# zprodev/zlib.es

Hardware: AMD Instinct MI355X
Metric: GiB/s deflate+inflate round trip, 64 MiB buffers (uncompressed bytes / wall), bit-exact vs reference (higher is better)
Workload: dtype u8; 1 GPU; random64: 1 x 64 MiB xorshift buffer(s) per GPU (seed 12345+index), deflate then inflate, HBM-resident; bytes_per_buffer=67108864, compressed_bytes=67176156, parallelism=independent buffers, one per GPU

## Files before the change

### zlib.es_amd/csrc/zes_api.hip

```cpp
#include "../../include/zes.h"
#include "zes_kernels.h"
#include "zes_chain.h"

#include <algorithm>
#include <atomic>
#include <condition_variable>
#include <cstdio>
#include <cstddef>
#include <cstdlib>
#include <cstring>
#include <chrono>
#include <functional>
#include <future>
#include <initializer_list>
#include <deque>
#include <map>
#include <mutex>
#include <string>
#include <thread>
#include <vector>

extern "C" int zes_gen(uint8_t* out, uint64_t n, uint32_t kind, uint32_t seed);

namespace {
// ... 694 lines not shown
                       ZES_SORT_MODE_FIRST | (use_index ? ZES_SORT_USE_INDEX : 0u));
  }
  auto note = [&](uint32_t* flag_to, uint32_t* word_to) -> int {
    HIPCHK(hipMemcpyAsync(flag_to, idx_a + ZES_BLK - 1, 4, hipMemcpyDeviceToHost, g.stream));
    if (word_to) HIPCHK(hipMemcpyAsync(word_to, idx_b + ZES_BLK - 1, 4, hipMemcpyDeviceToHost, g.stream));
    return ZES_OK;
  };
  if (route && (rc = note(&route[0], &route[3]))) return rc;
  if (use_index) {
    {
      Timed t("k_lz_index");
      hipLaunchKernelGGL(k_lz_index, dim3(grid), dim3(IDX_THREADS), 0, g.stream, d_in, dbufs, dblks, idx_a, idx_b, idx_a, (uint16_t*)g.sdelta.p);
    }
    if (route && (rc = note(&route[1], &route[4]))) return rc;
    {
      Timed t("k_lz_sort_redo");
      hipLaunchKernelGGL(k_lz_sort, dim3(grid), dim3(SORT_THREADS), 0, g.stream, d_in, dbufs, dblks, idx_a, idx_b, idx_a, (uint16_t*)g.sdelta.p,
                         ZES_SORT_MODE_REDO);
    }
    if (route && (rc = note(&route[2], nullptr))) return rc;
  }
  if ((rc = after_index())) return rc;
  {
    Timed t("k_lz_match");
    hipLaunchKernelGGL(k_lz_match, dim3(grid), dim3(MATCH_THREADS), 0, g.stream, d_in, dbufs, dblks, idx_a, idx_b, (uint32_t*)g.mlist.p);
  }
  if (phases && (rc = phases_arm(zes_lazy_set_dbg, grid))) return rc;
  {
    const uint32_t* order = nullptr;
    if (heaviest_first) {
      if ((rc = ensure(g.order, (size_t)grid * 4))) return rc;
      Timed t("k_lz_order");
      hipLaunchKernelGGL(k_lz_order, dim3(1), dim3(1024), 0, g.stream, (const uint32_t*)idx_a, grid, (uint32_t*)g.order.p);
      order = (const uint32_t*)g.order.p;
    }
    Timed t("k_lz_match_lazy");
    hipLaunchKernelGGL(k_lz_match_lazy, dim3(grid), dim3(MATCH_THREADS), 0, g.stream, d_in, dbufs, dblks, idx_a, (const uint32_t*)idx_a,
                       (const uint16_t*)g.sdelta.p, idx_b, (uint32_t*)g.tmask.p, (uint32_t*)g.mlist.p, order);
  }
  if (phases) {
    if ((rc = phases_print(zes_lazy_set_dbg, grid, 5,
                           "zes lazy match steps (avg cycles over %u blocks): stage %.0f tail %.0f window chains %.0f entry chains %.0f true chain (only unmerged blocks) %.0f | first wave, window chains: %.0f loop turns\n")))
      return rc;
    if ((rc = phases_arm(zes_parse_set_dbg, grid))) return rc;
  }
  {
    Timed t("k_lz_parse_small");
    hipLaunchKernelGGL(k_lz_parse_small, dim3(grid), dim3(PARSE_THREADS), 0, g.stream, d_in, dbufs, dblks, idx_b, idx_a, (uint32_t*)g.hists.p,
                       (const uint32_t*)g.tmask.p, (const uint32_t*)g.mlist.p);
  }
  {
    Timed t("k_lz_parse");
    hipLaunchKernelGGL(k_lz_parse, dim3(grid), dim3(PARSE_THREADS), 0, g.stream, d_in, dbufs, dblks, idx_b, idx_a, (uint32_t*)g.hists.p,
                       (const uint32_t*)g.tmask.p, (const uint32_t*)g.mlist.p);
  }
  return ZES_OK;
}

struct DeflateRange {
  uint64_t n_read = 0;
  uint32_t flags = 0;
  uint32_t start_bit = 0;
  bool defer = false;
  uint32_t adler = 1;
};

int deflate_batch_core(const uint8_t* d_in, const uint64_t* in_off, const uint64_t* in_len, uint8_t* d_out,
                       const uint64_t* out_off, const uint64_t* out_cap, uint64_t* out_len, int32_t* status,
                       uint32_t count, DeflateRange* one = nullptr) {
  std::vector<ZesBuf> hb;
  uint64_t nblk_total = 0;
  std::vector<uint32_t> live;
  hb.reserve(count);
  for (uint32_t i = 0; i < count; i++) {
    out_len[i] = 0;
    if (deflate_throws(in_len[i])) {
      status[i] = ZES_E_CORRUPT;
      continue;
    }
    if (out_cap[i] < deflate_bound(in_len[i])) {
      status[i] = ZES_E_NOSPACE;
      out_len[i] = deflate_bound(in_len[i]);
      continue;
    }
    if ((out_off[i] & 15u) || (((uintptr_t)d_out) & 15u)) {
      status[i] = ZES_E_ARG;
      continue;
    }
    status[i] = ZES_OK;
    ZesBuf b;
    b.in_off = in_off[i];
    b.n = in_len[i];
    b.out_off = out_off[i];
    b.cap = out_cap[i];
    b.first_blk = (uint32_t)nblk_total;
    b.nblk = (uint32_t)((in_len[i] + ZES_BLK - 1) / ZES_BLK);
    b.n_read = one ? std::max(one->n_read, in_len[i]) : in_len[i];
    b.flags = one ? one->flags : 0u;
    b.start_bit = one ? one->start_bit : 0u;
    nblk_total += b.nblk;
    hb.push_back(b);
    live.push_back(i);
  }
  if (hb.empty()) return ZES_OK;
  if (nblk_total >= (1ull << 31)) return ZES_E_ARG;
  const uint32_t nbuf = (uint32_t)hb.size(), nblk = (uint32_t)nblk_total;
  int rc;
  if ((rc = ensure(g.bufs, sizeof(ZesBuf) * nbuf))) return rc;
  if ((rc = ensure(g.blks, sizeof(ZesBlk) * nblk))) return rc;
  if ((rc = ensure(g.idx_a, (size_t)nblk * ZES_BLK * 4))) return rc;
  if ((rc = ensure(g.idx_b, (size_t)nblk * ZES_BLK * 4))) return rc;
  if ((rc = ensure(g.sdelta, (size_t)nblk * ZES_BLK * 2 + 64))) return rc;
  if ((rc = ensure(g.tmask, (size_t)nblk * ZES_TMASK_WORDS * 4))) return rc;
  if ((rc = ensure(g.mlist, (size_t)nblk * ZES_MLIST_WORDS * 4))) return rc;
  if ((rc = ensure(g.hists, (size_t)nblk * 320 * 4))) return rc;
  if ((rc = ensure(g.codes, (size_t)nblk * 320 * 4))) return rc;
  if ((rc = ensure(g.hdrs, (size_t)nblk * ZES_HDR_WORDS * 4))) return rc;
  if ((rc = ensure(g.adler, (size_t)nbuf * 16))) return rc;
  if ((rc = ensure(g.res, sizeof(ZesRes) * nbuf))) return rc;
  ZesBuf* dbufs = (ZesBuf*)g.bufs.p;
  ZesBlk* dblks = (ZesBlk*)g.blks.p;
  unsigned long long* adler = (unsigned long long*)g.adler.p;
  if (nbuf > 1) {
    if (nbuf <= DEFLATE_TABLE_BUFS) {
      memcpy(g.pinned->def.table, hb.data(), sizeof(ZesBuf) * nbuf);
      HIPCHK(hipMemcpyAsync(g.bufs.p, g.pinned->def.table, sizeof(ZesBuf) * nbuf, hipMemcpyHostToDevice, g.stream));
    } else {
      HIPCHK(hipMemcpy(g.bufs.p, hb.data(), sizeof(ZesBuf) * nbuf, hipMemcpyHostToDevice));
    }
  }
  {
    Timed t("k_make_blks");
    const uint32_t nthr = std::max(nblk, 2u * nbuf);
    hipLaunchKernelGGL(k_make_blks, dim3((nthr + 255) / 256), dim3(256), 0, g.stream, hb[0], nbuf, dbufs, dblks, nblk, adler);
  }
  {
    HIPCHK(hipEventRecord(g.ev_a0, g.stream));
    HIPCHK(hipStreamWaitEvent(g.s_adler, g.ev_a0, 0));
    Timed t("k_adler", g.s_adler);
    if (nbuf == 1) {
      const uint32_t nch = (uint32_t)((hb[0].n + ADLER_CHUNK - 1) / ADLER_CHUNK);
      hipLaunchKernelGGL(k_adler, dim3(nch), dim3(ADLER_THREADS), 0, g.s_adler, d_in, hb[0].in_off, hb[0].n, adler);
    } else {
      hipLaunchKernelGGL(k_adler_blocks, dim3(nblk), dim3(ADLER_THREADS), 0, g.s_adler, d_in, dbufs, dblks, adler);
    }
  }
  HIPCHK(hipEventRecord(g.ev_a1, g.s_adler));
  const bool sort_dbg = getenv("ZES_DEBUG_PHASES") != nullptr;
  if (sort_dbg && (rc = phases_arm(zes_sort_set_dbg, nblk))) return rc;
  static const bool use_index = getenv("ZES_NO_INDEX") == nullptr;
  rc = launch_lz77(d_in, nblk, use_index, nbuf > 1 && nblk > 256, sort_dbg, [&]() -> int {
    if (!sort_dbg) return ZES_OK;
    return phases_print(zes_sort_set_dbg, nblk, 7,
                        "zes sort steps (avg cycles over %u blocks): zero %.0f count %.0f flag %.0f compact %.0f stage %.0f three passes %.0f sd/inv %.0f\n");
  });
  if (rc) return rc;
  if (sort_dbg) {
    if ((rc = phases_print(zes_parse_set_dbg, nblk, 7, "zes parse steps (avg cycles over %u blocks): A %.0f B %.0f C %.0f D1 %.0f D2 %.0f D3 %.0f out %.0f\n"))) return rc;
    if ((rc = phases_arm(zes_huff_set_dbg, nblk))) return rc;
  }
  ZesRes* res_direct = (nbuf <= DEFLATE_DIRECT_BUFS && g.pinned_dev) ? g.pinned_dev->def.res : nullptr;
  {
    Timed t("k_huff");
    hipLaunchKernelGGL(k_huff, dim3(nblk), dim3(HUFF_THREADS_HOST), 0, g.stream, dblks, (const uint32_t*)g.hists.p,
                       (uint32_t*)g.codes.p, (uint32_t*)g.hdrs.p);
  }
  if (sort_dbg && (rc = phases_print(zes_huff_set_dbg, nblk, 7,
                                     "zes huff steps (avg cycles over %u blocks): rank sorts %.0f both alphabets' levels %.0f codes %.0f run-length coding %.0f its code %.0f header bits %.0f totals+out %.0f\n")))
    return rc;
  {
    HIPCHK(hipStreamWaitEvent(g.stream, g.ev_a1, 0));
    Timed t("k_layout");
    hipLaunchKernelGGL(k_layout, dim3(nbuf), dim3(256), 0, g.stream, d_out, dbufs, dblks, adler, res_direct ? res_direct : (ZesRes*)g.res.p);
  }
  {
    Timed t("k_emit");
    hipLaunchKernelGGL(k_emit, dim3(nblk), dim3(EMIT_THREADS), 0, g.stream, d_out, dbufs, dblks, (uint32_t*)g.idx_a.p,
                       (const uint32_t*)g.codes.p, (const uint32_t*)g.hdrs.p);
  }
  HIPCHK(hipGetLastError());
  ZesRes* r = g.pinned->def.res;
  if (nbuf > DEFLATE_DIRECT_BUFS) {
    if (nbuf > g.res_more_n) {
      if (g.res_more) HIPCHK(hipHostFree(g.res_more));
      g.res_more = nullptr;
      g.res_more_n = 0;
      HIPCHK(hipHostMalloc((void**)&g.res_more, sizeof(ZesRes) * nbuf * 2, hipHostMallocDefault));
      g.res_more_n = (size_t)nbuf * 2;
    }
    r = g.res_more;
  }
  if (!res_direct) HIPCHK(hipMemcpyAsync(r, g.res.p, sizeof(ZesRes) * nbuf, hipMemcpyDeviceToHost, g.stream));
  if (one && one->defer) return ZES_OK;
  HIPCHK(hipStreamSynchronize(g.stream));
  collect_times();
  for (uint32_t k = 0; k < nbuf; k++) {
    out_len[live[k]] = r[k].out_len;
    status[live[k]] = r[k].status;
  }
  if (one) one->adler = r[0].aux;
  return ZES_OK;
}

int deflate_one(const uint8_t* d_in, uint64_t in_off, uint64_t n, uint8_t* d_out, uint64_t out_off, uint64_t cap, uint64_t* out_len,
                DeflateRange* range = nullptr) {
  int32_t st = 0;
  const int rc = deflate_batch_core(d_in, &in_off, &n, d_out, &out_off, &cap, out_len, &st, 1, range);
  return rc ? rc : st;
}

int read_res(ZesRes* out) {
  HIPCHK(hipMemcpyAsync(&g.pinned->res1, g.res.p, sizeof(ZesRes), hipMemcpyDeviceToHost, g.stream));
  HIPCHK(hipStreamSynchronize(g.stream));
  *out = g.pinned->res1;
  return ZES_OK;
}

struct InfJob {
  uint64_t in_off, c, out_off, cap;
  uint64_t out_len;
  int status;
  int tier;
  uint32_t start0 = 16, hist = 0;
  bool partial = false, final_seen = false;
  uint64_t end_bit = 0;
  int btype0 = -1;
  bool want_end = false;
};

ZesInfBuf inf_buf(const InfJob& j) {
  ZesInfBuf b;
  memset(&b, 0, sizeof b);
  b.in_off = j.in_off;
  b.c = j.c;
  b.out_off = j.out_off;
  b.cap = j.cap;
  return b;
}

bool t1_eligible(const InfJob& j, uint32_t flags) { return !(flags & (ZES_F_NO_FASTPATH | ZES_F_PIECES)) && j.c >= 64 && j.c < (1ull << 29); }

int launch_verify(const uint8_t* d_in, const ZesInfBuf* dbufs, uint32_t surv_cap, uint32_t* counters, uint32_t* cnt, uint32_t loose,
                  uint64_t total_c) {
  int rc;
  const uint32_t vlong_cap = (uint32_t)std::min<uint64_t>(total_c / 256 + 4096, surv_cap);
  if ((rc = ensure(g.vlong, (size_t)vlong_cap * 24))) return rc;
  uint32_t nwg = (uint32_t)std::min<uint64_t>(total_c / 16384 + 1, 8192);
  if (const char* e = getenv("ZES_VERIFY_DIV")) nwg = (uint32_t)std::min<uint64_t>(total_c / (uint64_t)atoi(e) + 1, 8192);
  {
    Timed t("k_inf_verify");
    hipLaunchKernelGGL(k_inf_verify, dim3(nwg), dim3(64), 0, g.stream, d_in, dbufs, (const unsigned long long*)g.surv.p, surv_cap, counters,
                       (uint32_t*)g.cand.p, cnt, loose, (uint32_t*)g.vlong.p, vlong_cap,
                       getenv("ZES_VERIFY_STEPS") ? (uint32_t)atoi(getenv("ZES_VERIFY_STEPS")) : 32u);
  }
  {
    Timed t("k_inf_verify_long");
    const uint32_t nlong = (uint32_t)std::min<uint64_t>(total_c / 2048 + 1, 32768);
    hipLaunchKernelGGL(k_inf_verify_long, dim3(nlong), dim3(64), 0, g.stream, d_in, dbufs, (const unsigned long long*)g.surv.p, surv_cap,
                       counters, (uint32_t*)g.cand.p, cnt, loose, (const uint32_t*)g.vlong.p, vlong_cap);
  }
  if (getenv("ZES_VERIFY_DBG")) {
    uint32_t hc[4];
    HIPCHK(hipStreamSynchronize(g.stream));
    HIPCHK(hipMemcpy(hc, counters, 16, hipMemcpyDeviceToHost));
    fprintf(stderr, "verify: survivors %u, handed to the wave form %u\n", hc[0], hc[1]);
  }
  return ZES_OK;
}

void host_lap(const char* what) {
  static const bool on = getenv("ZES_DEBUG_HOSTLAPS") != nullptr;
  if (!on) return;
  static thread_local std::chrono::steady_clock::time_point last = std::chrono::steady_clock::now();
  const auto now = std::chrono::steady_clock::now();
  fprintf(stderr, "zes host lap: %-34s %8.1f us\n", what, std::chrono::duration<double, std::micro>(now - last).count());
  last = now;
}

int print_par_phases(const unsigned long long* dbg, uint64_t work) {
    std::vector<unsigned long long> h((size_t)work * ZES_PAR_DBG_ROW);
    HIPCHK(hipMemcpy(h.data(), dbg, h.size() * 8, hipMemcpyDeviceToHost));
    double acc[8] = {0}, t0[3] = {0}, t15[3] = {0}, fb_lanes = 0, fb_waves = 0, hs[5] = {0}, p4[5] = {0}, why[3] = {0};
    uint32_t cntd = 0;
    for (uint32_t i = 0; i < work; i++) {
      const unsigned long long* r = &h[(size_t)i * ZES_PAR_DBG_ROW];
      if (!r[7]) continue;
      cntd++;
      for (int k = 1; k < 8; k++) acc[k] += (double)(r[k] - r[k - 1]);
      for (int k = 0; k < 3; k++) {
        t0[k] += (double)(r[8 + k] - r[1]);
        t15[k] += (double)(r[12 + k] - r[1]);
      }
      hs[0] += (double)(r[16] - r[0]);
      for (int k = 1; k < 5; k++) hs[k] += (double)(r[16 + k] - r[15 + k]);
      for (int k = 0; k < 5; k++) p4[k] += (double)r[24 + k];
      fb_lanes += (double)r[11];
      fb_waves += (double)r[15];
      for (int k = 0; k < 3; k++) why[k] += (double)r[29 + k];
    }
    fprintf(stderr, "zes phases (avg cycles over %u blocks): hdr %.0f tables %.0f compose %.0f count %.0f emit %.0f resolve %.0f flush %.0f\n",
            cntd, acc[1] / cntd, acc[2] / cntd, acc[3] / cntd, acc[4] / cntd, acc[5] / cntd, acc[6] / cntd, acc[7] / cntd);
    fprintf(stderr, "zes table steps, cycles since the header: first wave window %.0f landing %.0f fill %.0f | last wave %.0f %.0f %.0f\n",
            t0[0] / cntd, t0[1] / cntd, t0[2] / cntd, t15[0] / cntd, t15[1] / cntd, t15[2] / cntd);
    fprintf(stderr, "zes header steps (avg cycles): staging %.0f fixed fields + code-length code %.0f code lengths %.0f lit/len tables %.0f distance tables %.0f\n",
            hs[0] / cntd, hs[1] / cntd, hs[2] / cntd, hs[3] / cntd, hs[4] / cntd);
    fprintf(stderr, "zes resolve steps (avg cycles): carry+clear %.0f fill %.0f jumping %.0f copy %.0f | %.1f barrier rounds per block\n", p4[0] / cntd,
            p4[1] / cntd, p4[2] / cntd, p4[3] / cntd, p4[4] / cntd);
// ... 4723 lines not shown
```

### zlib.es_amd/csrc/zes_deflate.hip

```cpp
#include "zes_common.h"
#include "zes_kernels.h"

__device__ static inline uint32_t lds_ld32u(const uint8_t* s, uint32_t off) {
  const uint32_t* w = reinterpret_cast<const uint32_t*>(s);
  uint32_t i = off >> 2;
  uint32_t lo = w[i], hi = w[i + 1];
  return __builtin_amdgcn_alignbyte(hi, lo, off & 3u);
}

__device__ static inline void stage_block(uint8_t* s, const uint8_t* g, uint32_t bytes, uint32_t padded) {
  const uint32_t tid = threadIdx.x, nth = blockDim.x;
  const uint32_t mis = (uint32_t)((uintptr_t)g & 15u);
  if (mis == 0) {
    const uint4* g4 = reinterpret_cast<const uint4*>(g);
    uint4* s4 = reinterpret_cast<uint4*>(s);
    const uint32_t full = bytes >> 4;
    for (uint32_t i = tid; i < full; i += nth) s4[i] = g4[i];
    for (uint32_t i = (full << 4) + tid; i < padded; i += nth) s[i] = i < bytes ? g[i] : (uint8_t)0;
  } else {
    for (uint32_t i = tid; i < padded; i += nth) s[i] = i < bytes ? g[i] : (uint8_t)0;
  }
}

__device__ unsigned long long* g_sort_dbg = nullptr;
void zes_sort_set_dbg(unsigned long long* p) { (void)hipMemcpyToSymbol(HIP_SYMBOL(g_sort_dbg), &p, sizeof p); }
#define SSTAMP(i)                                                                                        \
  do {                                                                                                   \
    if (g_sort_dbg && threadIdx.x == 0) g_sort_dbg[(size_t)blockIdx.x * 8 + (i)] = (unsigned long long)clock64(); \
  } while (0)

#define SORT_HASH_BITS 19u
#define SORT_OWN 128u
#ifndef SORT_ROUNDS
#define SORT_ROUNDS 8u
#endif
#define SORT_TILE (SORT_THREADS * SORT_ROUNDS)
static_assert(SORT_ROUNDS == 4u || SORT_ROUNDS == 8u || SORT_ROUNDS == 16u, "the arrival wait names four, eight or sixteen registers");
struct SortSmem {
  uint8_t in[ZES_BLK + 16];
  uint32_t hist[3][256];
  uint32_t base[2][256];
  uint16_t whist[2][SORT_WAVES][256];
  uint32_t wsum[SORT_WAVES];
  uint32_t nsat;
  uint32_t heavy;
};
static_assert((1u << SORT_HASH_BITS) * 2u / 8u <= ZES_BLK, "counter table must fit the block area");
static_assert(SORT_OWN * SORT_THREADS == ZES_BLK, "one thread per 128 positions");

__device__ __forceinline__ static uint32_t sort_hash(uint32_t key24) { return (key24 * 0x9E3779B1u) >> (32u - SORT_HASH_BITS); }
__device__ __forceinline__ static uint32_t sort_hash2(uint32_t key24) { return ((key24 ^ (key24 >> 11)) * 0xC2B2AE35u) >> (32u - SORT_HASH_BITS); }

__device__ __forceinline__ static uint4 sort_ld16(const uint8_t* __restrict__ src, bool aligned, uint32_t off, uint32_t T) {
  if (aligned && off + 16u <= T) return *reinterpret_cast<const uint4*>(src + off);
  uint32_t t[4] = {0, 0, 0, 0};
  for (uint32_t k = 0; k < 16u; k++)
    if (off + k < T) t[k >> 2] |= (uint32_t)src[off + k] << (8u * (k & 3u));
  return make_uint4(t[0], t[1], t[2], t[3]);
}

__global__ __launch_bounds__(SORT_THREADS) void k_lz_sort(const uint8_t* __restrict__ d_in, const ZesBuf* __restrict__ bufs,
                                                          const ZesBlk* __restrict__ blks, uint32_t* idx_a,
                                                          uint32_t* __restrict__ idx_b, uint32_t* inv_all, uint16_t* __restrict__ sd_all,
                                                          uint32_t mode) {
  __shared__ __align__(16) SortSmem S;
  const uint32_t g = blockIdx.x, tid = threadIdx.x, lane = tid & 63u, wave = tid >> 6;
  const ZesBlk bk = blks[g];
  const ZesBuf bf = bufs[bk.buf];
  const uint32_t T = bk.len;
  const uint8_t* src = d_in + bf.in_off + (uint64_t)bk.blk * ZES_BLK;
  uint32_t* A = idx_a + (uint64_t)g * ZES_BLK;
  uint32_t* B = idx_b + (uint64_t)g * ZES_BLK;
  const uint32_t cnt = T >= 3 ? T - 2 : 0;
  const bool redo = (mode & 0xffu) == ZES_SORT_MODE_REDO;
  if (redo && !(A[ZES_BLK - 1] & ZES_SORT_REDO)) return;
  if (cnt == 0) {
    if (tid == 0) A[ZES_BLK - 1] = 0;
    return;
  }

  SSTAMP(0);
  uint32_t* tbl = reinterpret_cast<uint32_t*>(S.in);
  {
    uint4* t4 = reinterpret_cast<uint4*>(S.in);
    for (uint32_t i = tid; i < ZES_BLK / 16; i += SORT_THREADS) t4[i] = make_uint4(0, 0, 0, 0);
    for (uint32_t i = tid; i < 4 * 3 * 256; i += SORT_THREADS) reinterpret_cast<uint32_t*>(&S.whist[0][0][0])[i] = 0;
    if (tid == 0) {
      S.nsat = 0;
      S.heavy = 0;
    }
  }
  __syncthreads();
  SSTAMP(1);
  const bool aligned = (((uintptr_t)src) & 15u) == 0;
  const uint32_t p0 = tid * SORT_OWN;
  uint32_t samp[SORT_OWN / 16];
#pragma unroll
  for (uint32_t c = 0; c < SORT_OWN / 16; c++) samp[c] = ~0u;
  if (p0 < cnt && !redo) {
    uint4 cur = sort_ld16(src, aligned, p0, T);
#pragma unroll 1
    for (uint32_t c = 0; c < SORT_OWN / 16; c++) {
      const uint4 nxt = sort_ld16(src, aligned, p0 + 16u * (c + 1u), T);
      const uint32_t w[5] = {cur.x, cur.y, cur.z, cur.w, nxt.x};
#pragma unroll
      for (uint32_t k = 0; k < 16; k++) {
        const uint32_t key = __builtin_amdgcn_alignbyte(w[(k >> 2) + 1], w[k >> 2], k & 3u) & 0xffffffu;
        const uint32_t h = sort_hash(key);
        const uint32_t sh = (h & 15u) * 2u;
        const bool inr = p0 + 16u * c + k < cnt;
        const bool sat = (tbl[h >> 4] >> sh) & 2u;
        if (k == 0 && inr) {
#pragma unroll
          for (uint32_t cc = 0; cc < SORT_OWN / 16; cc++) samp[cc] = (cc == c) ? h : samp[cc];
        }
        if (inr && !sat) {
          const uint32_t old = atomicOr(&tbl[h >> 4], 1u << sh);
          if (((old >> sh) & 3u) == 1u) atomicOr(&tbl[h >> 4], 2u << sh);
        }
      }
      cur = nxt;
    }
  }
  __syncthreads();
  SSTAMP(2);
  {
    uint32_t kept = 0, tried = 0;
#pragma unroll
    for (uint32_t c = 0; c < SORT_OWN / 16; c++) {
      const uint32_t h = samp[c];
      if (h != ~0u) {
        tried++;
        kept += (tbl[h >> 4] >> ((h & 15u) * 2u + 1u)) & 1u;
      }
    }
    atomicAdd(&S.nsat, kept | (tried << 16));
  }
  __syncthreads();
  const bool dense = redo || (S.nsat & 0xFFFFu) * 4u >= (S.nsat >> 16) * 3u;
#ifndef NO_LAZY
  if (dense && !redo && (mode & ZES_SORT_USE_INDEX) && inv_all != nullptr) {
    uint32_t* cc = reinterpret_cast<uint32_t*>(&S.whist[0][0][0]);
    {
      uint32_t ky[SORT_OWN / 16];
#pragma unroll
      for (uint32_t c = 0; c < SORT_OWN / 16; c++) {
        const uint32_t sp = min(p0 + 16u * c + (((tid * 8u + c) * 0x9E3779B1u) >> 28), T >= 8u ? T - 8u : 0u);
        uint32_t w = 0, w2 = 0;
        if (T >= 8u) {
          __builtin_memcpy(&w, src + (sp & ~3u), 4);
          __builtin_memcpy(&w2, src + (sp & ~3u) + 4u, 4);
        }
        ky[c] = __builtin_amdgcn_alignbyte(w2, w, sp & 3u) & 0xffffffu;
      }
#pragma unroll
      for (uint32_t c = 0; c < SORT_OWN / 16; c++)
        if (p0 + 16u * c < cnt) atomicAdd(&cc[sort_hash(ky[c]) >> (SORT_HASH_BITS - 11u)], 1u);
    }
    __syncthreads();
    {
      const uint32_t thr = max(2u, (32u * cnt + (ZES_BLK - 1u)) >> 17);
      const uint32_t a = cc[2u * tid], b = cc[2u * tid + 1u];
      const uint32_t w = (a > thr ? a : 0u) + (b > thr ? b : 0u);
      if (w) atomicAdd(&S.heavy, w);
    }
    __syncthreads();
    if (S.heavy * 256u <= cnt) {
      if (tid == 0) A[ZES_BLK - 1] = cnt | ZES_SORT_LAZY | ZES_SORT_INDEX;
      return;
    }
    cc[2u * tid] = 0;
    cc[2u * tid + 1u] = 0;
    __syncthreads();
  }
#endif
  const bool two = !redo && (S.nsat & 0xFFFFu) * 5u < (S.nsat >> 16) * 2u;
  if (tid == 0) B[ZES_BLK - 1] = (two ? ZES_ROUTE_SORT_TWO : 0u) | (dense ? ZES_ROUTE_SORT_DENSE : 0u);
  uint32_t ns = cnt;
  if (!dense) {
  uint32_t f0 = 0, f1 = 0, f2 = 0, f3 = 0;
  uint32_t(*sub)[256] = reinterpret_cast<uint32_t(*)[256]>(&S.whist[0][0][0]) + 3u * (lane & 3u);
  if (p0 < cnt) {
    uint4 cur = sort_ld16(src, aligned, p0, T);
#pragma unroll 1
    for (uint32_t c = 0; c < SORT_OWN / 16; c++) {
      const uint4 nxt = sort_ld16(src, aligned, p0 + 16u * (c + 1u), T);
      const uint32_t w[5] = {cur.x, cur.y, cur.z, cur.w, nxt.x};
      uint32_t bits = 0;
#pragma unroll
      for (uint32_t k = 0; k < 16; k++) {
        const uint32_t key = __builtin_amdgcn_alignbyte(w[(k >> 2) + 1], w[k >> 2], k & 3u) & 0xffffffu;
        const uint32_t h = sort_hash(key);
        const uint32_t keep = (tbl[h >> 4] >> ((h & 15u) * 2u + 1u)) & 1u;
        if (keep && p0 + 16u * c + k < cnt) {
          bits |= 1u << k;
          if (!two) {
            atomicAdd(&sub[0][(key >> 16) & 255u], 1u);
            atomicAdd(&sub[1][(key >> 8) & 255u], 1u);
            atomicAdd(&sub[2][key & 255u], 1u);
          }
        }
      }
      const uint32_t v = bits << (16u * (c & 1u));
      f0 |= (c >> 1) == 0u ? v : 0u;
      f1 |= (c >> 1) == 1u ? v : 0u;
      f2 |= (c >> 1) == 2u ? v : 0u;
      f3 |= (c >> 1) == 3u ? v : 0u;
      cur = nxt;
    }
  }
  if (two) {
    __syncthreads();
    {
      uint4* t4 = reinterpret_cast<uint4*>(S.in);
      for (uint32_t i = tid; i < ZES_BLK / 16; i += SORT_THREADS) t4[i] = make_uint4(0, 0, 0, 0);
    }
    __syncthreads();
    if (p0 < cnt) {
      uint4 cur = sort_ld16(src, aligned, p0, T);
#pragma unroll 1
      for (uint32_t c = 0; c < SORT_OWN / 16; c++) {
        const uint4 nxt = sort_ld16(src, aligned, p0 + 16u * (c + 1u), T);
        const uint32_t w[5] = {cur.x, cur.y, cur.z, cur.w, nxt.x};
        const uint32_t fw = (c >> 1) == 0u ? f0 : (c >> 1) == 1u ? f1 : (c >> 1) == 2u ? f2 : f3;
        const uint32_t bits = (fw >> (16u * (c & 1u))) & 0xffffu;
#pragma unroll
        for (uint32_t k = 0; k < 16; k++) {
          const uint32_t key = __builtin_amdgcn_alignbyte(w[(k >> 2) + 1], w[k >> 2], k & 3u) & 0xffffffu;
          const uint32_t h = sort_hash2(key);
          const uint32_t sh = (h & 15u) * 2u;
          if ((bits >> k) & 1u) {
            const uint32_t old = atomicOr(&tbl[h >> 4], 1u << sh);
            if (((old >> sh) & 3u) == 1u) atomicOr(&tbl[h >> 4], 2u << sh);
          }
        }
        cur = nxt;
      }
    }
    __syncthreads();
    if (p0 < cnt) {
      uint32_t g0 = 0, g1 = 0, g2 = 0, g3 = 0;
      uint4 cur = sort_ld16(src, aligned, p0, T);
#pragma unroll 1
      for (uint32_t c = 0; c < SORT_OWN / 16; c++) {
        const uint4 nxt = sort_ld16(src, aligned, p0 + 16u * (c + 1u), T);
        const uint32_t w[5] = {cur.x, cur.y, cur.z, cur.w, nxt.x};
        const uint32_t fw = (c >> 1) == 0u ? f0 : (c >> 1) == 1u ? f1 : (c >> 1) == 2u ? f2 : f3;
        const uint32_t bits = (fw >> (16u * (c & 1u))) & 0xffffu;
        uint32_t nb = 0;
#pragma unroll
        for (uint32_t k = 0; k < 16; k++) {
          const uint32_t key = __builtin_amdgcn_alignbyte(w[(k >> 2) + 1], w[k >> 2], k & 3u) & 0xffffffu;
          const uint32_t h = sort_hash2(key);
          const uint32_t keep = (tbl[h >> 4] >> ((h & 15u) * 2u + 1u)) & 1u;
          if (keep && ((bits >> k) & 1u)) {
            nb |= 1u << k;
            atomicAdd(&sub[0][(key >> 16) & 255u], 1u);
            atomicAdd(&sub[1][(key >> 8) & 255u], 1u);
            atomicAdd(&sub[2][key & 255u], 1u);
          }
        }
        const uint32_t v = nb << (16u * (c & 1u));
        g0 |= (c >> 1) == 0u ? v : 0u;
        g1 |= (c >> 1) == 1u ? v : 0u;
        g2 |= (c >> 1) == 2u ? v : 0u;
        g3 |= (c >> 1) == 3u ? v : 0u;
        cur = nxt;
      }
      f0 = g0;
      f1 = g1;
      f2 = g2;
      f3 = g3;
    }
  }
  SSTAMP(3);
  const uint32_t mine = (uint32_t)(__popc(f0) + __popc(f1) + __popc(f2) + __popc(f3));
  uint32_t incl = mine;
#pragma unroll
  for (int d = 1; d < 64; d <<= 1) {
    const uint32_t t = __shfl_up(incl, d);
    if ((int)lane >= d) incl += t;
  }
  if (lane == 63) S.wsum[wave] = incl;
  __syncthreads();
  uint32_t woff = 0;
  ns = 0;
#pragma unroll
  for (uint32_t w = 0; w < SORT_WAVES; w++) {
    const uint32_t v = S.wsum[w];
    woff += w < wave ? v : 0u;
    ns += v;
  }
  uint32_t* fbits = reinterpret_cast<uint32_t*>(S.in);
  uint32_t* fpre = reinterpret_cast<uint32_t*>(S.in) + 4096;
  if (two) {
    uint32_t o = woff + incl - mine;
#pragma unroll
    for (uint32_t w = 0; w < 4; w++) {
      uint32_t f = w == 0u ? f0 : w == 1u ? f1 : w == 2u ? f2 : f3;
      while (f) {
        B[o++] = p0 + 32u * w + (uint32_t)__builtin_ctz(f);
        f &= f - 1u;
      }
    }
  } else {
    uint32_t o = woff + incl - mine;
    fbits[4 * tid + 0] = f0;
    fpre[4 * tid + 0] = o;
    o += (uint32_t)__popc(f0);
    fbits[4 * tid + 1] = f1;
    fpre[4 * tid + 1] = o;
    o += (uint32_t)__popc(f1);
    fbits[4 * tid + 2] = f2;
    fpre[4 * tid + 2] = o;
    o += (uint32_t)__popc(f2);
    fbits[4 * tid + 3] = f3;
    fpre[4 * tid + 3] = o;
  }
  if (tid < 3 * 256) {
    const uint32_t* hs = reinterpret_cast<const uint32_t*>(&S.whist[0][0][0]);
    (&S.hist[0][0])[tid] = hs[tid] + hs[768 + tid] + hs[1536 + tid] + hs[2304 + tid];
  }
  __syncthreads();
  if (!two) {
    for (uint32_t p = tid; p < cnt; p += SORT_THREADS) {
      const uint32_t w = fbits[p >> 5];
      if ((w >> (p & 31u)) & 1u) B[fpre[p >> 5] + (uint32_t)__popc(w & ((1u << (p & 31u)) - 1u))] = p;
    }
  }
  }
  __syncthreads();
  SSTAMP(4);
#ifdef NO_LAZY
  const bool lazy = false;
#else
  const bool lazy = inv_all != nullptr && ns * 2u >= cnt;
#endif
  if (tid == 0) A[ZES_BLK - 1] = ns | (lazy ? ZES_SORT_LAZY : 0u);
  if (ns == 0) return;

  stage_block(S.in, src, T, (T + 15u) & ~15u);
  __syncthreads();
  if (dense) {
    uint32_t(*hc)[256] = reinterpret_cast<uint32_t(*)[256]>(&S.whist[0][0][0]);
    for (uint32_t i = tid; i < T; i += SORT_THREADS) atomicAdd(&hc[lane & 3u][S.in[i]], 1u);
    __syncthreads();
    if (tid < 256) {
      const uint32_t H = hc[0][tid] + hc[1][tid] + hc[2][tid] + hc[3][tid];
#pragma unroll
      for (uint32_t ps = 0; ps < 3; ps++) {
        const uint32_t off = 2u - ps;
        uint32_t h = H;
        for (uint32_t e = 0; e < off; e++) h -= (S.in[e] == tid);
        for (uint32_t e = off + cnt; e < T; e++) h -= (S.in[e] == tid);
        S.hist[ps][tid] = h;
      }
    }
    __syncthreads();
  }
  SSTAMP(5);

  uint32_t bsel = 0;
  for (int pass = 0; pass < 3; pass++) {
    const uint32_t off = 2u - (uint32_t)pass;
    const uint32_t* from = (pass == 1) ? A : B;
    uint32_t* to = (pass == 1) ? B : A;
    {
      uint32_t* w0 = reinterpret_cast<uint32_t*>(&S.whist[0][wave][0]);
      w0[lane] = 0;
      w0[lane + 64u] = 0;
    }
    if (wave == 0) {
      uint32_t c[4];
      uint32_t sum = 0;
#pragma unroll
      for (int k = 0; k < 4; k++) {
        c[k] = S.hist[pass][lane * 4 + k];
        sum += c[k];
      }
      uint32_t in2 = sum;
#pragma unroll
      for (int d = 1; d < 64; d <<= 1) {
        const uint32_t t = __shfl_up(in2, d);
        if ((int)lane >= d) in2 += t;
      }
      uint32_t run = in2 - sum;
#pragma unroll
      for (int k = 0; k < 4; k++) {
        S.base[bsel][lane * 4 + k] = run;
        run += c[k];
      }
    }
    __syncthreads();
    const uint32_t ntiles = (ns + SORT_TILE - 1) / SORT_TILE;
    uint32_t pn[SORT_ROUNDS];
#pragma unroll
    for (uint32_t r = 0; r < SORT_ROUNDS; r++) pn[r] = from[min(wave * (SORT_TILE / SORT_WAVES) + lane + 64u * r, ns - 1u)];
    for (uint32_t t = 0; t < ntiles; t++) {
      uint16_t(*wh)[256] = S.whist[t & 1];
      const uint32_t i0 = t * SORT_TILE + wave * (SORT_TILE / SORT_WAVES) + lane;
      uint32_t p[SORT_ROUNDS], d[SORT_ROUNDS], rk[SORT_ROUNDS];
#pragma unroll
      for (uint32_t r = 0; r < SORT_ROUNDS; r++) p[r] = (dense && pass == 0) ? min(i0 + 64u * r, ns - 1u) : pn[r];
      asm volatile("" : "+v"(p[0]), "+v"(p[1]), "+v"(p[2]), "+v"(p[3]));
#if SORT_ROUNDS >= 8u
      asm volatile("" : "+v"(p[4]), "+v"(p[5]), "+v"(p[6]), "+v"(p[7]));
#endif
#if SORT_ROUNDS == 16u
      asm volatile("" : "+v"(p[8]), "+v"(p[9]), "+v"(p[10]), "+v"(p[11]));
      asm volatile("" : "+v"(p[12]), "+v"(p[13]), "+v"(p[14]), "+v"(p[15]));
#endif
#pragma unroll
      for (uint32_t r = 0; r < SORT_ROUNDS; r++) d[r] = (i0 + 64u * r < ns) ? S.in[p[r] + off] : 0u;
      uint32_t* wrow = reinterpret_cast<uint32_t*>(&wh[wave][0]);
#pragma unroll
      for (uint32_t r = 0; r < SORT_ROUNDS; r++) {
        const bool valid = i0 + 64u * r < ns;
        const uint32_t sh = 16u * (d[r] & 1u);
        const uint32_t old = valid ? atomicAdd(&wrow[d[r] >> 1], 1u << sh) : 0u;
        rk[r] = (old >> sh) & 0xffffu;
      }
      __syncthreads();
      if (tid < 256) {
        uint32_t c[SORT_WAVES];
#pragma unroll
        for (int w = 0; w < SORT_WAVES; w++) c[w] = wh[w][tid];
        uint32_t o = 0;
#pragma unroll
        for (int w = 0; w < SORT_WAVES; w++) {
          wh[w][tid] = (uint16_t)o;
          o += c[w];
        }
        S.base[bsel ^ 1][tid] = S.base[bsel][tid] + o;
      }
      __syncthreads();
      {
        uint32_t* wnext = reinterpret_cast<uint32_t*>(&S.whist[(t + 1u) & 1u][wave][0]);
        wnext[lane] = 0;
        wnext[lane + 64u] = 0;
      }
#pragma unroll
      for (uint32_t r = 0; r < SORT_ROUNDS; r++) pn[r] = from[min(i0 + SORT_TILE + 64u * r, ns - 1u)];
#pragma unroll
      for (uint32_t r = 0; r < SORT_ROUNDS; r++) {
        const uint32_t dst = S.base[bsel][d[r]] + wh[wave][d[r]] + rk[r];
        const bool valid = i0 + 64u * r < ns;
        to[valid ? dst : ZES_BLK - 2u] = p[r];
      }
      bsel ^= 1;
    }
    __syncthreads();
    SSTAMP(6);
  }
  if (lazy) {
    uint32_t* inv = inv_all + (uint64_t)g * ZES_BLK;
    uint16_t* sd = sd_all + (uint64_t)g * ZES_BLK;
    uint32_t* P = B;
    uint32_t* pcur = S.wsum;
    static_assert(SORT_WAVES >= 8, "eight bucket cursors live in wsum[]");
    if (tid < 8u) pcur[tid] = 0;
    __syncthreads();
    for (uint32_t rb = tid; rb < ns; rb += 8u * SORT_THREADS) {
      uint32_t pos[8], prv[8];
#pragma unroll
      for (uint32_t k = 0; k < 8; k++) {
        const uint32_t r = min(rb + k * SORT_THREADS, ns - 1u);
        pos[k] = A[r];
        prv[k] = A[r ? r - 1u : 0u];
      }
      asm volatile("" : "+v"(pos[0]), "+v"(pos[1]), "+v"(pos[2]), "+v"(pos[3]), "+v"(pos[4]), "+v"(pos[5]), "+v"(pos[6]), "+v"(pos[7]));
      asm volatile("" : "+v"(prv[0]), "+v"(prv[1]), "+v"(prv[2]), "+v"(prv[3]), "+v"(prv[4]), "+v"(prv[5]), "+v"(prv[6]), "+v"(prv[7]));
#pragma unroll
      for (uint32_t k = 0; k < 8; k++) {
        const uint32_t r = rb + k * SORT_THREADS;
        const bool valid = r < ns;
        const uint32_t key = valid ? (lds_ld32u(S.in, pos[k]) & 0xffffffu) : 0u;
        uint32_t kprev = (uint32_t)__shfl_up((int)key, 1);
        if (lane == 0 && valid) kprev = lds_ld32u(S.in, prv[k]) & 0xffffffu;
        const bool sm = valid && r != 0u && key == kprev;
        const uint32_t delta = pos[k] - prv[k];
        const bool has = sm && delta <= ZES_WINDOW;
        const uint32_t sl = pos[k] >> 14;
// ... 2243 lines not shown
```

Before: 47.10 GiB/s.

## Compact level-1 survivors into a list for second-level hash and sort

In the two-level sort path of k_lz_sort, positions that survive the first hash level are compacted into a 16-bit position list in shared memory, so the second hash level only processes survivors instead of rescanning all positions. When the final survivor count fits a tile, a three-pass radix sort runs in shared memory and writes the result straight to the output, skipping the global intermediate. This adds considerable code, register pressure and extra barriers. On random input few positions survive, so the benefit depends on how often the listed path triggers.

```diff
diff --git a/zlib.es_amd/csrc/zes_api.hip b/zlib.es_amd/csrc/zes_api.hip
--- a/zlib.es_amd/csrc/zes_api.hip
+++ b/zlib.es_amd/csrc/zes_api.hip
@@ -870,7 +870,7 @@
   rc = launch_lz77(d_in, nblk, use_index, nbuf > 1 && nblk > 256, sort_dbg, [&]() -> int {
     if (!sort_dbg) return ZES_OK;
     return phases_print(zes_sort_set_dbg, nblk, 7,
-                        "zes sort steps (avg cycles over %u blocks): zero %.0f count %.0f flag %.0f compact %.0f stage %.0f three passes %.0f sd/inv %.0f\n");
+                        "zes sort steps (avg cycles over %u blocks): zero %.0f count %.0f flags %.0f level 2 + compact %.0f stage %.0f three passes %.0f sd/inv %.0f\n");
   });
   if (rc) return rc;
   if (sort_dbg) {
diff --git a/zlib.es_amd/csrc/zes_deflate.hip b/zlib.es_amd/csrc/zes_deflate.hip
--- a/zlib.es_amd/csrc/zes_deflate.hip
+++ b/zlib.es_amd/csrc/zes_deflate.hip
@@ -59,6 +59,15 @@
   return make_uint4(t[0], t[1], t[2], t[3]);
 }
 
+__device__ __forceinline__ static uint32_t sort_key_at(const uint32_t* __restrict__ srcw, uint32_t mis, uint32_t p) {
+  const uint32_t o = p + mis, s = o & 3u;
+  return __builtin_amdgcn_alignbyte(srcw[(o >> 2) + (s >= 2u ? 1u : 0u)], srcw[o >> 2], s) & 0xffffffu;
+}
+
+#define SORT_LIST_WORDS 16u
+#define SORT_LIST_CAP (SORT_THREADS * SORT_LIST_WORDS * 2u)
+static_assert(SORT_LIST_CAP * 4u <= ZES_BLK, "the final list of positions, one word each, lives in the block area");
+
 __global__ __launch_bounds__(SORT_THREADS) void k_lz_sort(const uint8_t* __restrict__ d_in, const ZesBuf* __restrict__ bufs,
                                                           const ZesBlk* __restrict__ blks, uint32_t* idx_a,
                                                           uint32_t* __restrict__ idx_b, uint32_t* inv_all, uint16_t* __restrict__ sd_all,
@@ -93,6 +102,8 @@
   __syncthreads();
   SSTAMP(1);
   const bool aligned = (((uintptr_t)src) & 15u) == 0;
+  const uint32_t mis4 = (uint32_t)((uintptr_t)src & 3u);
+  const uint32_t* srcw = reinterpret_cast<const uint32_t*>(src - mis4);
   const uint32_t p0 = tid * SORT_OWN;
   uint32_t samp[SORT_OWN / 16];
 #pragma unroll
@@ -209,8 +220,250 @@
       cur = nxt;
     }
   }
+  SSTAMP(3);
+  bool listed = false;
+  uint32_t n1 = 0, nlo = 0, at1 = 0;
   if (two) {
-    __syncthreads();
+    const uint32_t mine1 = (uint32_t)(__popc(f0) + __popc(f1) + __popc(f2) + __popc(f3));
+    uint32_t incl1 = mine1;
+#pragma unroll
+    for (int d = 1; d < 64; d <<= 1) {
+      const uint32_t t = __shfl_up(incl1, d);
+      if ((int)lane >= d) incl1 += t;
+    }
+    if (lane == 63) S.wsum[wave] = incl1;
+    __syncthreads();
+    at1 = incl1 - mine1;
+#pragma unroll
+    for (uint32_t w = 0; w < SORT_WAVES; w++) {
+      const uint32_t v = S.wsum[w];
+      at1 += w < wave ? v : 0u;
+      nlo += w < SORT_WAVES / 2u ? v : 0u;
+      n1 += v;
+    }
+    listed = n1 <= SORT_LIST_CAP;
+  }
+  if (listed) {
+    uint32_t e[SORT_LIST_WORDS];
+    {
+      uint16_t* l16 = reinterpret_cast<uint16_t*>(S.in);
+      uint32_t o = at1;
+#pragma unroll
+      for (uint32_t w = 0; w < 4; w++) {
+        uint32_t f = w == 0u ? f0 : w == 1u ? f1 : w == 2u ? f2 : f3;
+        while (f) {
+          l16[o++] = (uint16_t)(p0 + 32u * w + (uint32_t)__builtin_ctz(f));
+          f &= f - 1u;
+        }
+      }
+    }
+    __syncthreads();
+    const uint32_t nwords = (n1 + 1u) >> 1;
+    const uint32_t wshare = (nwords + SORT_WAVES - 1u) / SORT_WAVES;
+#pragma unroll
+    for (uint32_t j = 0; j < SORT_LIST_WORDS; j++) e[j] = tbl[min(wave * wshare + 64u * j + lane, nwords ? nwords - 1u : 0u)];
+#define SORT_LIST_ENTRY(j, k, pos, valid)                                              \
+  const uint32_t li_ = 2u * (wave * wshare + 64u * (j) + lane) + (k);                  \
+  const bool valid = 64u * (j) + lane < wshare && li_ < n1;                            \
+  const uint32_t pos = valid ? ((e[j] >> (16u * (k))) & 0xffffu) + (li_ >= nlo ? 65536u : 0u) : 0u
+    uint32_t hh[2u * SORT_LIST_WORDS];
+#pragma unroll
+    for (uint32_t q0 = 0; q0 < 2u * SORT_LIST_WORDS; q0 += SORT_LIST_WORDS) {
+#pragma unroll
+      for (uint32_t q = q0; q < q0 + SORT_LIST_WORDS; q++) {
+        SORT_LIST_ENTRY(q >> 1, q & 1u, pos, valid);
+        const uint32_t key = sort_key_at(srcw, mis4, pos);
+        hh[q] = valid ? sort_hash2(key) : ~0u;
+      }
+#pragma unroll
+      for (uint32_t q = q0; q < q0 + SORT_LIST_WORDS; q += 4u) asm volatile("" : "+v"(hh[q]), "+v"(hh[q + 1u]), "+v"(hh[q + 2u]), "+v"(hh[q + 3u]));
+    }
+    __syncthreads();
+    {
+      uint4* t4 = reinterpret_cast<uint4*>(S.in);
+      for (uint32_t i = tid; i < ZES_BLK / 16; i += SORT_THREADS) t4[i] = make_uint4(0, 0, 0, 0);
+    }
+    __syncthreads();
+#pragma unroll
+    for (uint32_t g8 = 0; g8 < 2u * SORT_LIST_WORDS; g8 += 8u) {
+      if (32u * g8 < wshare) {
+        uint32_t old[8];
+#pragma unroll
+        for (uint32_t q = 0; q < 8; q++) {
+          const bool valid = hh[g8 + q] != ~0u;
+          const uint32_t h = valid ? hh[g8 + q] : tid * 16u, sh = (h & 15u) * 2u;
+          old[q] = atomicOr(&tbl[h >> 4], valid ? 1u << sh : 0u);
+        }
+#pragma unroll
+        for (uint32_t q = 0; q < 8; q++) {
+          const bool valid = hh[g8 + q] != ~0u;
+          const uint32_t h = valid ? hh[g8 + q] : tid * 16u, sh = (h & 15u) * 2u;
+          atomicOr(&tbl[h >> 4], (valid && ((old[q] >> sh) & 3u) == 1u) ? 2u << sh : 0u);
+        }
+      }
+    }
+    __syncthreads();
+    uint32_t vb = 0;
+#pragma unroll
+    for (uint32_t q = 0; q < 2u * SORT_LIST_WORDS; q++) {
+      const bool valid = hh[q] != ~0u;
+      const uint32_t h = valid ? hh[q] : 0u;
+      const uint32_t keep = (tbl[h >> 4] >> ((h & 15u) * 2u + 1u)) & 1u;
+      vb |= (valid ? keep : 0u) << q;
+    }
+    uint32_t wtot = (uint32_t)__popc(vb);
+#pragma unroll
+    for (int d = 32; d >= 1; d >>= 1) wtot += __shfl_xor(wtot, d);
+    if (lane == 0) S.wsum[wave] = wtot;
+    __syncthreads();
+    uint32_t run = 0;
+    ns = 0;
+#pragma unroll
+    for (uint32_t w = 0; w < SORT_WAVES; w++) {
+      const uint32_t v = S.wsum[w];
+      run += w < wave ? v : 0u;
+      ns += v;
+    }
+    uint32_t* fin = reinterpret_cast<uint32_t*>(S.in);
+#pragma unroll
+    for (uint32_t j = 0; j < SORT_LIST_WORDS; j++) {
+      if (64u * j < wshare) {
+        const uint32_t b0 = (vb >> (2u * j)) & 1u, b1 = (vb >> (2u * j + 1u)) & 1u;
+        const uint64_t m0 = __ballot(b0), m1 = __ballot(b1);
+        const uint32_t at = run + (uint32_t)__popcll(m0 & zes_lanemask_lt()) + (uint32_t)__popcll(m1 & zes_lanemask_lt());
+        if (b0) {
+          SORT_LIST_ENTRY(j, 0u, pos, valid);
+          (void)valid;
+          fin[at] = pos;
+        }
+        if (b1) {
+          SORT_LIST_ENTRY(j, 1u, pos, valid);
+          (void)valid;
+          fin[at + b0] = pos;
+        }
+        run += (uint32_t)__popcll(m0) + (uint32_t)__popcll(m1);
+      }
+    }
+#undef SORT_LIST_ENTRY
+    __syncthreads();
+#ifdef NO_LAZY
+    const bool lazy_l = false;
+#else
+    const bool lazy_l = inv_all != nullptr && ns * 2u >= cnt;
+#endif
+    if (ns != 0u && ns <= SORT_TILE && !lazy_l) {
+      static_assert(SORT_TILE * 8u <= ZES_BLK, "a tile's keys and positions fit the block area");
+      uint32_t* lkey = reinterpret_cast<uint32_t*>(S.in);
+      uint32_t* lpos = lkey + SORT_TILE;
+      const uint32_t i0 = wave * (SORT_TILE / SORT_WAVES) + lane;
+      uint32_t kk[SORT_ROUNDS], pp[SORT_ROUNDS], rk[SORT_ROUNDS];
+#pragma unroll
+      for (uint32_t r = 0; r < SORT_ROUNDS; r++) pp[r] = fin[min(i0 + 64u * r, ns - 1u)];
+#pragma unroll
+      for (uint32_t r = 0; r < SORT_ROUNDS; r++) kk[r] = sort_key_at(srcw, mis4, pp[r]);
+#pragma unroll
+      for (uint32_t r = 0; r < SORT_ROUNDS; r++) {
+        if (i0 + 64u * r < ns) {
+          atomicAdd(&sub[0][(kk[r] >> 16) & 255u], 1u);
+          atomicAdd(&sub[1][(kk[r] >> 8) & 255u], 1u);
+          atomicAdd(&sub[2][kk[r] & 255u], 1u);
+        }
+      }
+      if (tid == 0) A[ZES_BLK - 1] = ns;
+      __syncthreads();
+      SSTAMP(4);
+      if (tid < 3 * 256) {
+        const uint32_t* hs = reinterpret_cast<const uint32_t*>(&S.whist[0][0][0]);
+        (&S.hist[0][0])[tid] = hs[tid] + hs[768 + tid] + hs[1536 + tid] + hs[2304 + tid];
+      }
+      __syncthreads();
+      if (wave < 3u) {
+        uint32_t c[4];
+        uint32_t sum = 0;
+#pragma unroll
+        for (int k = 0; k < 4; k++) {
+          c[k] = S.hist[wave][lane * 4 + k];
+          sum += c[k];
+        }
+        uint32_t in2 = sum;
+#pragma unroll
+        for (int d = 1; d < 64; d <<= 1) {
+          const uint32_t t = __shfl_up(in2, d);
+          if ((int)lane >= d) in2 += t;
+        }
+        uint32_t run2 = in2 - sum;
+#pragma unroll
+        for (int k = 0; k < 4; k++) {
+          S.hist[wave][lane * 4 + k] = run2;
+          run2 += c[k];
+        }
+      }
+      uint32_t* wrow = reinterpret_cast<uint32_t*>(&S.whist[0][wave][0]);
+      wrow[lane] = 0;
+      wrow[lane + 64u] = 0;
+      __syncthreads();
+      SSTAMP(5);
+      for (uint32_t pass = 0; pass < 3u; pass++) {
+        const uint32_t dsh = 16u - 8u * pass;
+        if (pass) {
+#pragma unroll
+          for (uint32_t r = 0; r < SORT_ROUNDS; r++) {
+            const uint32_t i = min(i0 + 64u * r, ns - 1u);
+            kk[r] = lkey[i];
+            pp[r] = lpos[i];
+          }
+        }
+#pragma unroll
+        for (uint32_t r = 0; r < SORT_ROUNDS; r++) {
+          const uint32_t d = (kk[r] >> dsh) & 255u, sh = 16u * (d & 1u);
+          const uint32_t old = (i0 + 64u * r < ns) ? atomicAdd(&wrow[d >> 1], 1u << sh) : 0u;
+          rk[r] = (old >> sh) & 0xffffu;
+        }
+        __syncthreads();
+        if (tid < 256) {
+          uint32_t o = 0;
+#pragma unroll
+          for (int w = 0; w < SORT_WAVES; w++) {
+            const uint32_t c = S.whist[0][w][tid];
+            S.whist[0][w][tid] = (uint16_t)o;
+            o += c;
+          }
+        }
+        __syncthreads();
+#pragma unroll
+        for (uint32_t r = 0; r < SORT_ROUNDS; r++) {
+          const uint32_t d = (kk[r] >> dsh) & 255u;
+          const uint32_t dst = S.hist[pass][d] + S.whist[0][wave][d] + rk[r];
+          if (i0 + 64u * r < ns) {
+            lkey[dst] = kk[r];
+            lpos[dst] = pp[r];
+          }
+        }
+        wrow[lane] = 0;
+        wrow[lane + 64u] = 0;
+        __syncthreads();
+      }
+      SSTAMP(6);
+      for (uint32_t i = tid; i < ns; i += SORT_THREADS) A[i] = lpos[i];
+      SSTAMP(7);
+      return;
+    }
+    for (uint32_t i = tid; i < ns; i += SORT_THREADS) {
+      const uint32_t pos = fin[i];
+      const uint32_t key = sort_key_at(srcw, mis4, pos);
+      B[i] = pos;
+      atomicAdd(&sub[0][(key >> 16) & 255u], 1u);
+      atomicAdd(&sub[1][(key >> 8) & 255u], 1u);
+      atomicAdd(&sub[2][key & 255u], 1u);
+    }
+    asm volatile("s_waitcnt vmcnt(0)" ::: "memory");
+    __syncthreads();
+    if (tid < 3 * 256) {
+      const uint32_t* hs = reinterpret_cast<const uint32_t*>(&S.whist[0][0][0]);
+      (&S.hist[0][0])[tid] = hs[tid] + hs[768 + tid] + hs[1536 + tid] + hs[2304 + tid];
+    }
+  } else {
+  if (two) {
     {
       uint4* t4 = reinterpret_cast<uint4*>(S.in);
       for (uint32_t i = tid; i < ZES_BLK / 16; i += SORT_THREADS) t4[i] = make_uint4(0, 0, 0, 0);
@@ -273,7 +526,6 @@
       f3 = g3;
     }
   }
-  SSTAMP(3);
   const uint32_t mine = (uint32_t)(__popc(f0) + __popc(f1) + __popc(f2) + __popc(f3));
   uint32_t incl = mine;
 #pragma unroll
@@ -328,6 +580,9 @@
       if ((w >> (p & 31u)) & 1u) B[fpre[p >> 5] + (uint32_t)__popc(w & ((1u << (p & 31u)) - 1u))] = p;
     }
   }
+  }
+  } else {
+    SSTAMP(3);
   }
   __syncthreads();
   SSTAMP(4);
```

Result: faster. 49.67 GiB/s (median of 6 runs) (+5.5%).
